# Wil-Lee/NN_BVH

Measured on AMD Instinct MI355X. Metric: Mray/s (closest-hit + any-hit), higher is better.
Workload: dtype f32; 1 GPU; crown, 1000x1400: one wavefront pass of 8 spp per step (8 spp per GPU-film) — primary, bounce-1 and bounce-2 closest-hit, shadow any-hit towards the light quads (batches pre-generated, hence independent: ONE launch; the dependent form is dependent_step), rays in --ray-order tile (a caller-side order the reference's integrator does not form: ray_order_probe), RecordShadowRayResult + RGBFilm::AddSam; sample_sets=4, geometry=procedural stand-in for crown (3548192 tris; data/crown.npz absent), tree=sah, triangles=3548192, nodes=7032259, rays_primary=11200000, rays_bounce=7410327, rays_bounce2=4392209, parallelism=tile-sharded x1, BVH replicated, film all-gather after the pass

## Files before the change

### nn_bvh_amd/aggregate.py

```python
import ctypes

import numpy as np

from . import _lib
from ._lib import HIT_DTYPE, NODE_DTYPE, PRIM_DTYPE, RAY_DTYPE, NNBVHError, check, ptr

SPLIT_METHODS = {"sah": 0, "hlbvh": 1, "middle": 2, "equal": 3}


def make_prims(tri_indices=None, patch_indices=None):
    nt = 0 if tri_indices is None else len(tri_indices)
    npch = 0 if patch_indices is None else len(patch_indices)
    prims = np.zeros(nt + npch, PRIM_DTYPE)
    prims["id"] = np.arange(nt + npch, dtype=np.int32)
    if nt:
        prims["kind"][:nt] = 0
        prims["v"][:nt, :3] = np.asarray(tri_indices, np.int32).reshape(nt, 3)
    if npch:
        prims["kind"][nt:] = 1
        prims["v"][nt:] = np.asarray(patch_indices, np.int32).reshape(npch, 4)
    return prims


def make_rays(o, d, tmax=np.inf, time=0.0):
# ... 313 lines not shown
            self.normals = np.ascontiguousarray(normals, np.float32).reshape(-1, 3)
            assert len(self.normals) == len(self.verts)
            self._h = L.nnbvh_scene_create_with_normals(ptr(self.nodes), len(self.nodes), ptr(self.ordered_prims),
                                                        len(self.ordered_prims), ptr(self.verts), ptr(self.normals),
                                                        len(self.verts), self.device)
        else:
            self._h = L.nnbvh_scene_create(ptr(self.nodes), len(self.nodes), ptr(self.ordered_prims),
                                           len(self.ordered_prims), ptr(self.verts), len(self.verts),
                                           self.device)
        if not self._h:
            raise NNBVHError("nnbvh_scene_create: " + _lib.last_error())
        self._read_info()

    def close(self):
        if getattr(self, "_h", None):
            _lib.lib().nnbvh_scene_destroy(self._h)
            self._h = None

    def __del__(self):
        try:
            self.close()
        except Exception:
            pass

    def set_option(self, key, value):
        check(_lib.lib().nnbvh_scene_set_option(self._h, key.encode(), int(value)),
              f"set_option({key})")

    def sched_stats(self, reset=True):
        out = np.zeros(16, np.uint64)
        check(_lib.lib().nnbvh_scene_sched_stats(self._h, ptr(out), int(reset)), "sched_stats")
        return dict(zip(("int_trips", "int_lanes", "prim_trips", "prim_lanes", "refill_trips",
                         "refill_lanes", "i_nint", "i_nprim", "i_nidle", "spare0", "int_cycles",
                         "prim_cycles", "refill_cycles", "spare1", "int_steps", "int_step_lanes"),
                        (int(x) for x in out)))

    def Bounds(self):
        out = np.zeros(6, np.float32)
        check(_lib.lib().nnbvh_scene_bounds(self._h, ptr(out)), "nnbvh_scene_bounds")
        return out[:3].copy(), out[3:].copy()

    def Intersect(self, rays, out=None):
        rays = np.ascontiguousarray(rays, RAY_DTYPE)
        hits = np.zeros(len(rays), HIT_DTYPE) if out is None else out
        assert hits.dtype == HIT_DTYPE and len(hits) == len(rays) and hits.flags.c_contiguous
        check(_lib.lib().nnbvh_intersect_closest(self._h, ptr(rays), len(rays), ptr(hits)),
              "nnbvh_intersect_closest")
        return hits

    def IntersectP(self, rays, counts=False):
        rays = np.ascontiguousarray(rays, RAY_DTYPE)
        occ = np.zeros(len(rays), np.uint8)
        if counts:
            vis = np.zeros(len(rays), np.int32)
            tst = np.zeros(len(rays), np.int32)
            check(_lib.lib().nnbvh_intersect_any(self._h, ptr(rays), len(rays), ptr(occ),
                                                 ptr(vis), ptr(tst)), "nnbvh_intersect_any")
            return occ, vis, tst
        check(_lib.lib().nnbvh_intersect_any(self._h, ptr(rays), len(rays), ptr(occ), None, None),
              "nnbvh_intersect_any")
        return occ

    def intersect_device(self, d_rays, d_hits, n, stream=0):
        check(_lib.lib().nnbvh_intersect_closest_device(self._h, d_rays, n, d_hits, stream),
              "nnbvh_intersect_closest_device")

    def trace_batches_device(self, batches, stream=0):
# ... 141 lines not shown
```

### nn_bvh_amd/build.py

```python
import concurrent.futures
import hashlib
import os
import shutil
import subprocess

HERE = os.path.dirname(os.path.abspath(__file__))
CSRC = os.path.join(HERE, "csrc")
LIB = os.path.join(HERE, "libnnbvh_hip.so")
SOURCES = ["bvh_trace.hip", "wavefront.hip", "wavefront2.hip", "wavefront_items.hip", "bvh_build_gpu.hip", "bvh_bake.hip", "interaction.hip", "film.hip", "kd_trace.hip", "kd_build_gpu.hip", "kd_bake.hip", "bvh_capi.cpp", "capi_two_level.cpp", "capi_trace.cpp", "capi_kd.cpp", "capi_wavefront.cpp", "capi_shading.cpp", "bvh_build.cpp", "kd_build.cpp"]
HEADERS = ["bvh_trace.h", "trace_instance.h", "trace_math.h", "stream_access.h", "spawn_math.h", "anim_math.h", "alpha_texture_math.h", "wavefront2.h", "walk_math.h", "wavefront.h", "bvh_build_gpu.h", "interaction.h", "interaction_math.h", "wavefront_items.h", "kd_trace.h", "kd_build_gpu.h", "kd_device_util.h", "nnbvh_internal.h", "capi_internal.h", os.path.join("..", "..", "include", "nnbvh.h")]
CFLAGS = ["-O3", "--offload-arch=gfx950", "-ffp-contract=off", "-fPIC", "-std=c++17",
          "-Wall", "-Wno-unused-function", "-Wno-pass-failed"]
FLAGS = CFLAGS + ["-shared"]


def _hipcc():
    hipcc = shutil.which("hipcc") or "/opt/rocm/bin/hipcc"
    if not os.path.exists(hipcc):
        raise RuntimeError("hipcc not found: cannot build libnnbvh_hip.so")
    return hipcc


def _sources():
    return [s for s in SOURCES if os.path.exists(os.path.join(CSRC, s))]


def _deps_mtime():
    deps = [os.path.join(CSRC, f) for f in HEADERS] + [os.path.abspath(__file__)]
    return max(os.path.getmtime(d) for d in deps if os.path.exists(d))


def _stale():
    if not os.path.exists(LIB):
        return True
    t = os.path.getmtime(LIB)
    return _deps_mtime() > t or any(os.path.getmtime(os.path.join(CSRC, s)) > t for s in _sources())


def _build(out, extra=(), force=False, verbose=False, jobs=None):
    hipcc = _hipcc()
    tag = hashlib.sha1(" ".join(extra).encode()).hexdigest()[:10] if extra else "product"
    objdir = os.path.join(HERE, "_obj", tag)
    os.makedirs(objdir, exist_ok=True)
# ... 43 lines not shown
```

### nn_bvh_amd/csrc/bvh_capi.cpp

```cpp
#include <algorithm>
#include <cmath>
#include <cstring>
#include <limits>
#include <vector>

#include "alpha_texture_math.h"
#include "bvh_build_gpu.h"
#include "capi_internal.h"

namespace nnbvh {

static thread_local std::string g_error;
void set_error(const std::string &msg) { g_error = msg; }

}

using namespace nnbvh;

static bool validate_tree(const nnbvh_linear_node *nodes, int root, int n_tree, const nnbvh_prim *prims,
                          int n_prims, bool allow_instances, std::vector<uint8_t> &covered,
                          std::vector<uint8_t> &leaf_last, int *depth_out) {
    if (n_tree < 1) {
        set_error("scene_create: tree has no nodes");
        return false;
    }
    const int n_nodes = root + n_tree;
    struct Frame {
        int node, end, depth;
    };
    std::vector<Frame> st;
    st.push_back({root, n_nodes, 0});
    int visited = 0, max_depth = 0;
    while (!st.empty()) {
        Frame f = st.back();
        st.pop_back();
        ++visited;
        if (f.node < 0 || f.node >= f.end) {
            set_error("scene_create: node index outside its subtree range");
            return false;
        }
        max_depth = std::max(max_depth, f.depth);
// ... 126 lines not shown
        AlphaTexDesc &d = table[(size_t)k];
        d.texelLo = (uint32_t)total;
        d.texelHi = (uint32_t)(total >> 32);
        d.width = t.width;
        d.height = t.height;
        d.wrap = t.wrap;
        d.pointFilter = t.point_filter ? 1 : 0;
        d.su = t.su, d.sv = t.sv, d.du = t.du, d.dv = t.dv;
        d.scale = t.scale;
        d.invert = t.invert ? 1 : 0;
        total += (uint64_t)t.width * (uint64_t)t.height;
    }
    DeviceGuard guard(s->device);
    bool ok = guard.ok && hip_ok(hipMalloc((void **)&s->d_alpha_tex, table.size() * sizeof(AlphaTexDesc)), "hipMalloc(alpha textures)") &&
              hip_ok(hipMalloc((void **)&s->d_alpha_texels, (size_t)total * 4), "hipMalloc(alpha texels)") &&
              hip_ok(hipMemcpy(s->d_alpha_tex, table.data(), table.size() * sizeof(AlphaTexDesc), hipMemcpyHostToDevice),
                     "hipMemcpy(alpha textures)");
    uint64_t at = 0;
    for (int k = 0; ok && k < n_textures; ++k) {
        const uint64_t n = (uint64_t)textures[k].width * (uint64_t)textures[k].height;
        ok = hip_ok(hipMemcpy(s->d_alpha_texels + at, textures[k].texels, (size_t)n * 4, hipMemcpyHostToDevice),
                    "hipMemcpy(alpha texels)");
        at += n;
    }
    if (!ok) {
        const std::string why = nnbvh_last_error();
        nnbvh_scene_destroy(s);
        set_error(why);
        return false;
    }
    s->n_alpha_tex = n_textures;
    s->n_alpha_texels = (int64_t)total;
    s->device_bytes += table.size() * sizeof(AlphaTexDesc) + (size_t)total * 4;
    return true;
}

extern "C" {

const char *nnbvh_last_error(void) { return g_error.c_str(); }

int nnbvh_device_count(void) {
    int n = 0;
    if (hipGetDeviceCount(&n) != hipSuccess) return 0;
    return n;
}

static nnbvh_scene *scene_from_baked(const BakedScene &b, int depth, int device) {
    hipDeviceProp_t prop;
    if (!hip_ok(hipGetDeviceProperties(&prop, device), "hipGetDeviceProperties")) {
        (void)hipFree(b.d_wide);
        return nullptr;
    }
    auto *s = new nnbvh_scene;
    s->device = device;
    s->n_cus = prop.multiProcessorCount;
    s->n_interior = b.n_interior;
    s->n_slots = b.n_slots;
    s->depth = depth;
    std::memcpy(s->bounds, b.bounds, sizeof b.bounds);
    s->root_ref = b.root_ref;
    s->instanced = 0;
    s->has_host_prims = (b.has_host_prims || b.has_alpha) ? 1 : 0;
    s->has_patches = (b.has_patches || b.has_alpha) ? 1 : 0;
    s->has_alpha = b.has_alpha;
    s->max_grid_threads = s->n_cus * 8 * kBlockThreads;
    s->d_wide = (float4 *)b.d_wide;
    s->d_prims = (float4 *)b.d_prims;
    s->device_bytes = (size_t)std::max(b.n_interior, 1) * sizeof(WideNode) +
                      std::max<size_t>((size_t)b.n_slots, 1) * 16;
    if (hipMalloc((void **)&s->d_stats, 16 * sizeof(unsigned long long)) == hipSuccess)
        (void)hipMemset(s->d_stats, 0, 16 * sizeof(unsigned long long));
    return s;
}

static nnbvh_scene *create_scene_device_bake(const nnbvh_linear_node *nodes, int n_nodes, const nnbvh_prim *prims,
                                             int n_prims, const float *verts, int n_verts, int depth, int device,
                                             const float *normals, const float *prim_alpha, const float *uvs) {
    int n_dev = nnbvh_device_count();
    if (n_dev <= 0 || device < 0 || device >= n_dev) {
        set_error("scene_create: no usable HIP device (this library has no CPU fallback)");
        return nullptr;
    }
    DeviceGuard guard(device);
    if (!guard.ok) return nullptr;
    void *d_nodes = nullptr, *d_prims = nullptr, *d_verts = nullptr, *d_normals = nullptr, *d_alpha = nullptr,
         *d_uvs = nullptr;
    const size_t nb = (size_t)n_nodes * sizeof(nnbvh_linear_node), pbytes = (size_t)n_prims * sizeof(nnbvh_prim),
                 vb = (size_t)n_verts * 12;
    BakedScene b;
    std::string err;
    bool ok = hip_ok(hipMalloc(&d_nodes, nb), "hipMalloc(tree)") && hip_ok(hipMalloc(&d_prims, pbytes), "hipMalloc(primitives)") &&
              hip_ok(hipMalloc(&d_verts, vb), "hipMalloc(vertices)") &&
              hip_ok(hipMemcpy(d_nodes, nodes, nb, hipMemcpyHostToDevice), "hipMemcpy(tree)") &&
              hip_ok(hipMemcpy(d_prims, prims, pbytes, hipMemcpyHostToDevice), "hipMemcpy(primitives)") &&
              hip_ok(hipMemcpy(d_verts, verts, vb, hipMemcpyHostToDevice), "hipMemcpy(vertices)");
    if (ok && normals)
        ok = hip_ok(hipMalloc(&d_normals, vb), "hipMalloc(normals)") &&
             hip_ok(hipMemcpy(d_normals, normals, vb, hipMemcpyHostToDevice), "hipMemcpy(normals)");
    if (ok && prim_alpha)
        ok = hip_ok(hipMalloc(&d_alpha, (size_t)n_prims * 4), "hipMalloc(primitive alpha)") &&
             hip_ok(hipMemcpy(d_alpha, prim_alpha, (size_t)n_prims * 4, hipMemcpyHostToDevice), "hipMemcpy(primitive alpha)");
    if (ok && uvs)
        ok = hip_ok(hipMalloc(&d_uvs, (size_t)n_verts * 8), "hipMalloc(uvs)") &&
             hip_ok(hipMemcpy(d_uvs, uvs, (size_t)n_verts * 8, hipMemcpyHostToDevice), "hipMemcpy(uvs)");
// ... 435 lines not shown
}

void nnbvh_scene_destroy(nnbvh_scene *s) {
    if (!s) return;
    DeviceGuard guard(s->device);
    (void)hipDeviceSynchronize();
    for (auto &kv : s->workspaces) {
        Workspace &w = kv.second;
        void *ptrs[] = {w.queue, w.spill, w.d_in, w.d_out, w.d_aux0, w.d_aux1, w.d_hits};
        for (void *p : ptrs)
            if (p) (void)hipFree(p);
        for (void *p : w.scratch)
            if (p) (void)hipFree(p);
    }
    for (HostSlot &sl : s->host_slots) {
        for (void *p : {sl.d_in, sl.d_out[0], sl.d_out[1], sl.d_out[2]})
            if (p) (void)hipFree(p);
        for (void *p : {sl.h_in, sl.h_out[0], sl.h_out[1], sl.h_out[2]})
            if (p) (void)hipHostFree(p);
        for (hipEvent_t e : {sl.ev_in, sl.ev_traced, sl.ev_out})
            if (e) (void)hipEventDestroy(e);
    }
    for (hipStream_t st : {s->host_up, s->host_trace, s->host_down})
        if (st) (void)hipStreamDestroy(st);
    for (int k = 0; k < nnbvh_scene::kSideStreams; ++k) {
        if (s->side[k]) (void)hipStreamDestroy(s->side[k]);
        if (s->ev_join[k]) (void)hipEventDestroy(s->ev_join[k]);
    }
    if (s->ev_fork) (void)hipEventDestroy(s->ev_fork);
    (void)hipFree(s->d_wide);
    if (s->d_anim) (void)hipFree(s->d_anim);
    if (s->d_alpha_tex) (void)hipFree(s->d_alpha_tex);
    if (s->d_alpha_texels) (void)hipFree(s->d_alpha_texels);
    if (s->d_stats) (void)hipFree(s->d_stats);
    delete s;
}

int nnbvh_scene_bounds(const nnbvh_scene *s, float out[6]) {
    if (!s || !out) {
        set_error("scene_bounds: null argument");
        return NNBVH_ERR_ARG;
    }
    std::memcpy(out, s->bounds, sizeof s->bounds);
    return NNBVH_OK;
}

int nnbvh_scene_info(const nnbvh_scene *s, int64_t out[6]) {
    if (!s || !out) {
        set_error("scene_info: null argument");
        return NNBVH_ERR_ARG;
    }
    out[0] = s->n_interior;
    out[1] = s->n_slots;
    out[2] = s->depth;
    out[3] = (int64_t)s->device_bytes;
    out[4] = grid_blocks(const_cast<nnbvh_scene *>(s), 0);
    out[5] = s->window;
    return NNBVH_OK;
}

int nnbvh_scene_read(const nnbvh_scene *s, int what, void *out, size_t bytes) {
    if (!s || !out) {
        set_error("scene_read: null argument");
        return NNBVH_ERR_ARG;
    }
    if (what < 0 || what > 4) {
// ... 64 lines not shown
    std::string k(key);
    if (k == "stack_window") {
        if (value != 4 && value != 8 && value != 16) {
            set_error("set_option: stack_window must be 4, 8 or 16");
            return NNBVH_ERR_ARG;
        }
        s->window = value;
    } else if (k == "blocks_per_cu") {
        if (value < 0 || value > 8) {
            set_error("set_option: blocks_per_cu must be 0..8");
            return NNBVH_ERR_ARG;
        }
        s->blocks_per_cu = value;
    } else if (k == "int_repeat") {
        if (value < 1 || value > 16) {
            set_error("set_option: int_repeat must be 1..16");
            return NNBVH_ERR_ARG;
        }
        s->int_repeat = value;
    } else if (k == "host_chunk") {
        if (value < 1024) {
            set_error("set_option: host_chunk must be at least 1024 rays");
            return NNBVH_ERR_ARG;
        }
        s->host_chunk = value;
    } else if (k == "prim_repeat") {
        if (value < 1 || value > 16) {
            set_error("set_option: prim_repeat must be 1..16");
            return NNBVH_ERR_ARG;
        }
        s->prim_repeat = value;
    } else if (k == "fused_batches") {
        s->fused_batches = value ? 1 : 0;
    } else if (k == "xcd_queues") {
        s->xcd_queues = value ? 1 : 0;
    } else if (k == "prim_weight") {
        if (value < 1 || value > 64) {
            set_error("set_option: prim_weight must be 1..64");
            return NNBVH_ERR_ARG;
        }
        s->prim_weight = value;
    } else if (k == "refill_weight") {
        if (value < 1 || value > 64) {
            set_error("set_option: refill_weight must be 1..64");
            return NNBVH_ERR_ARG;
        }
        s->refill_weight = value;
    } else {
        set_error("set_option: unknown key");
        return NNBVH_ERR_ARG;
    }
    return NNBVH_OK;
}

}

Workspace *nnbvh::workspace_for(nnbvh_scene *s, hipStream_t stream) {
    auto it = s->workspaces.find(stream);
    if (it != s->workspaces.end()) return &it->second;
    Workspace w;
    const size_t spill_bytes = (size_t)std::max(s->depth - 2, 1) * (size_t)s->max_grid_threads * sizeof(uint2);
    if (!hip_ok(hipMalloc((void **)&w.queue, kMaxFusedBatches * kMaxQueues * kQueueStrideWords * sizeof(unsigned)),
                "hipMalloc(queue)"))
        return nullptr;
    if (!hip_ok(hipMalloc((void **)&w.spill, spill_bytes), "hipMalloc(spill)")) {
        (void)hipFree(w.queue);
// ... 5 lines not shown
```

### nn_bvh_amd/csrc/bvh_trace.h

```cpp
#pragma once
#include <hip/hip_runtime.h>
#include <stdint.h>

#include "../../include/nnbvh.h"
#include "nnbvh_internal.h"
#include "trace_instance.h"
#include "walk_math.h"

namespace nnbvh {

constexpr int kBlockThreads = 256;
constexpr int kMaxQueues = 8;
constexpr int kQueueStrideWords = 32;
constexpr int kMaxFusedBatches = 4;
constexpr int kFusedIndexBits = 28;

struct TraceParams {
    const float4 *wide;
    const float4 *prims;
    float rootMin[3], rootMax[3];
    int rootRef;
    const nnbvh_ray *rays;
    nnbvh_hit *hits;
    uint8_t *occluded;
// ... 4 lines not shown
    unsigned *queue;
    int nQueues;
    int primWeight;
    int refillWeight;
    int hasHostPrims;
    int intRepeat;
    int primRepeat;
    int fits32;
    unsigned long long *stats;
    uint2 *spill;
    const float *anim;
    int nBatches;
    unsigned anyMask;
    const nnbvh_ray *bRays[kMaxFusedBatches];
    void *bOut[kMaxFusedBatches];
    long bN[kMaxFusedBatches];
    const int32_t *bNDev[kMaxFusedBatches];
    nnbvh_ray_soa soa;
    nnbvh_ray_soa bSoa[kMaxFusedBatches];
    int hcCap;
    int32_t *hcCount;
    int32_t *hcBefore;
    int32_t *hcPrim;
    int32_t *hcInst;
    int bHcCap[kMaxFusedBatches];
    int32_t *bHcCount[kMaxFusedBatches];
    int32_t *bHcBefore[kMaxFusedBatches];
    int32_t *bHcPrim[kMaxFusedBatches];
    int32_t *bHcInst[kMaxFusedBatches];
    ShadingMeshDevice wMesh;
    WalkParams walk;
    const float4 *alphaTex;
    const float *alphaTexels;
};

hipError_t launch_zero_queue(unsigned *queue, int words, hipStream_t stream);
hipError_t launch_zero_words(int32_t *words, long n, int maxBlocks, hipStream_t stream);

hipError_t launch_trace(const TraceInstance &is, const TraceParams &p, int blocks, hipStream_t stream, int *occupancy);

}
```

### nn_bvh_amd/csrc/bvh_trace.hip

```cpp
#include <hip/hip_runtime.h>
#include <stdint.h>
#include <array>
#include <cstring>
#include <utility>

#include "bvh_trace.h"
#include "alpha_texture_math.h"
#include "anim_math.h"
#include "spawn_math.h"
#include "stream_access.h"
#include "trace_math.h"
#include "walk_math.h"

namespace nnbvh {

constexpr int kDone = (int)0x80000000;
constexpr int kReturn = (int)0x80000001;
constexpr int kEnter = (int)0x80000002;

#ifndef NNBVH_MINW_CLOSEST
#define NNBVH_MINW_CLOSEST 6
#endif
#ifndef NNBVH_MINW_ANY
#define NNBVH_MINW_ANY 6
// ... 16 lines not shown
#ifndef NNBVH_MINW_WALK
#define NNBVH_MINW_WALK 4
#endif
constexpr int min_waves(int modew, int inst, int patch, int alpha) {
    if (inst) return 1;
    if (modew >= 4) return patch ? NNBVH_MINW_WALK : NNBVH_MINW_WALK_LEAN;
    if (alpha == 2) return NNBVH_MINW_ALPHA_PATCH;
    if (alpha == 3) return NNBVH_MINW_ALPHA_TEX;
    if (alpha) return NNBVH_MINW_ALPHA;
    return ((modew == 0 || modew == 3) ? NNBVH_MINW_CLOSEST : NNBVH_MINW_ANY) + (patch ? 0 : NNBVH_LEAN_EXTRA_WAVES);
}
#ifndef NNBVH_ANIM_ENTER_WEIGHT
#define NNBVH_ANIM_ENTER_WEIGHT 8
#endif
template <typename T>
__device__ __forceinline__ T pick_batch(const T (&a)[kMaxFusedBatches], int b) {
    static_assert(kMaxFusedBatches == 4, "written out for four batches");
    return b == 0 ? a[0] : (b == 1 ? a[1] : (b == 2 ? a[2] : a[3]));
}

#define BVH_BEGIN_RAY(R0, R1)                                                                                         \
    do {                                                                                                              \
        r.o = {(R0).x, (R0).y, (R0).z};                                                                               \
        tMax = (R0).w;                                                                                                \
        const V3 d = {(R1).x, (R1).y, (R1).z};                                                                        \
        if (PATCH) {                                                                                                  \
            cold[kColdD][lane] = d.x;                                                                                 \
            cold[kColdD + 1][lane] = d.y;                                                                             \
            cold[kColdD + 2][lane] = d.z;                                                                             \
        }                                                                                                             \
                                                                                          \
        r.inv = {1.0f / d.x, 1.0f / d.y, 1.0f / d.z};                                                                 \
        ray_shear(r, d);                                                                                              \
        if (MODE == 0 || MODE == 3) {                                                                                 \
            cold[kColdHit][lane] = __int_as_float(-1);                                                                \
            cold[kColdHit + 1][lane] = 0.0f;                                                                          \
            cold[kColdHit + 2][lane] = 0.0f;                                                                          \
            cold[kColdHit + 3][lane] = 0.0f;                                                                          \
        }                                                                                                             \
        if (INST) {                                                                                                   \
            cold[kHitInst][lane] = 0.0f;                                                                              \
            cold[kCurInst][lane] = 0.0f;                                                                              \
            cold[kColdTime][lane] = (R1).w;                                 \
            floor = -1;                                                                                               \
        }                                                                                                             \
        if (!kLean && (HOSTC || p.hasHostPrims)) cold[kColdHost][lane] = 0.0f;           \
        if constexpr (WALK != 0) {                                                                                    \
            cold[kWalkD][lane] = (R1).x;                                                                              \
            cold[kWalkD + 1][lane] = (R1).y;                                                                          \
            cold[kWalkD + 2][lane] = (R1).z;                                                                          \
            cold[kWalkTime][lane] = (R1).w;                                                                           \
            cold[kWalkTMax][lane] = (R0).w;                                                                           \
        }                                                                                                             \
        visited = 1;                                                                                    \
        tests = 0;                                                                                                    \
        found = false;                                                                                                \
        sp = base = 0;                                                                                                \
        float tEntry;                                                                                                 \
        const bool rootHit = slab_partial(p.rootMin[0], p.rootMin[1], p.rootMin[2], p.rootMax[0], p.rootMax[1],       \
                                          p.rootMax[2], r, tEntry) &&                                                 \
                             (tEntry < tMax);                                                                         \
        cur = rootHit ? p.rootRef : kDone;                                                                            \
    } while (0)

template <int MODEW, int W, int INST, int PATCH, int ALPHA = 0, int SOA = 0, int HOSTC = 0>
__global__ __launch_bounds__(kBlockThreads, min_waves(MODEW, INST, PATCH, ALPHA))
void trace_kernel(TraceParams p) {
    constexpr int WALK = MODEW >= 4 ? MODEW - 3 : 0;
    constexpr int MODE = WALK ? 0 : MODEW;
    static_assert(!WALK || (MODEW <= 5 && W == 8 && INST != 2 && !ALPHA && !SOA && !HOSTC),
                  "walk instances: the plain record-reading closest-hit form at window 8");
    static_assert(PATCH || !INST, "two-level scenes need the ray direction");
    static_assert(PATCH || !ALPHA, "the alpha test hashes the ray direction");
    static_assert(ALPHA != 3 || (INST == 0 && W == 8 && MODE != 3), "textured alpha: flat scenes, window 8, modes 0 / 1 / 2");
    static_assert(!HOSTC || (PATCH && (MODE == 0 || MODE == 2 || (MODE == 3 && !ALPHA && W == 8)) && !SOA),
                  "candidate mode: general instances of modes 0 / 2 / 3");
    __shared__ float s_stack[kBlockThreads / 64][W][2][64];
    constexpr bool kLean = !PATCH && !INST;
    constexpr int kColdRi = 0, kColdD = 1, kColdHit = kLean ? 0 : (PATCH ? 4 : 1),
                  kColdHost = kColdHit + ((MODE == 0 || MODE == 3) ? 4 : 0);
    constexpr int kColdBase = kColdHost + (kLean ? 0 : 1);
    constexpr int kSaveO = kColdBase, kSaveInv = kColdBase + 3, kSaveShear = kColdBase + 6,
                  kSaveKz = kColdBase + 9, kSaveTmax = kColdBase + 10, kSaveD = kColdBase + 11,
                  kResume = kColdBase + 14, kCurInst = kColdBase + 15, kHitInst = kColdBase + 16,
                  kInnerHit = kColdBase + 17, kColdTime = kColdBase + 18, kPendSlot = kColdBase + 19;
    constexpr int kColdWalk = kColdBase + (INST ? 20 : 0);
    [[maybe_unused]] constexpr int kWalkD = kColdWalk, kWalkTime = kColdWalk + 3, kWalkTMax = kColdWalk + 4,
                                   kWalkCalls = kColdWalk + 5;
    constexpr int kColdFields = kColdWalk + (WALK ? 6 : 0);
    __shared__ float s_cold[kBlockThreads / 64][kColdFields > 0 ? kColdFields : 1][64];

    const int lane = threadIdx.x & 63;
    const int wave = threadIdx.x >> 6;
    const int gtid = blockIdx.x * kBlockThreads + threadIdx.x;
    float(*stk)[2][64] = s_stack[wave];
    float(*cold)[64] = s_cold[wave];
    int riReg = -1;
    if (!kLean) cold[kColdRi][lane] = __int_as_float(-1);
    const long spillStride = (long)gridDim.x * kBlockThreads;

    int q = 0;
    if (p.nQueues > 1) {
        unsigned xcc;
        asm volatile("s_getreg_b32 %0, hwreg(HW_REG_XCC_ID)" : "=s"(xcc));
        q = (int)(xcc & 0xf) % p.nQueues;
    }
    int queuesTried = 0;
    int curBatch = 0;
    long nRays = p.n;
    if (p.nDev) {
        const long nd = (long)*p.nDev;
        nRays = nd < 0 ? 0 : (nd < nRays ? nd : nRays);
    }

#ifdef NNBVH_STATS
    unsigned long long st[16] = {0, 0, 0, 0, 0, 0, 0, 0, 0, 0, 0, 0, 0, 0, 0, 0};
    unsigned long long stPrev = __builtin_amdgcn_s_memtime();
    int stKind = 2;
#endif
    RayState r;
    RayMasks masks = {0ull, 0ull, 0ull, 0ull, 0ull, 0ull};
    float tMax = 0.0f;
    int visited = 0, tests = 0;
    int cur = kDone, sp = 0, base = 0;
    int floor = -1;
    bool found = false;
    bool exhausted = false;

    auto pop_entry = [&](int &ref, float &key) {
// ... 188 lines not shown
                        const float u = (a <= 0) ? 1.f : hash_float_6f(rn.o, rd);
                        if (!(u > a)) break;
                        if (k == kAlphaPatchDepth) {
                            hit = false;
                            cold[kColdHost][lane] = HOSTC ? __int_as_float(-2) : 1.0f;
                            break;
                        }
                        if (k == 0) t0 = th;
                        else if (k == 1) t1 = th;
                        else t2 = th;
                        ++k;
                        rn.o = patch_retrace_origin({s0.x, s0.y, s0.z}, {s1.x, s1.y, s1.z}, {s2.x, s2.y, s2.z},
                                                    {s3.x, s3.y, s3.z}, x0, x1, (flags & kPrimFlipN) != 0, rd,
                                                    (flags & kPrimSmooth) != 0, (flags & kPrimUV) != 0,
                                                    p.prims + slot + 4);
                        tm = tm - th;
                        tests += 1;
                    }
                    if (hit && k > 0) {
                        if (k == 3) th = th + t2;
                        if (k >= 2) th = th + t1;
                        th = th + t0;
                    }
                } else {
                    hit = patch_test(r, rd, tMax, {s0.x, s0.y, s0.z}, {s1.x, s1.y, s1.z},
                                     {s2.x, s2.y, s2.z}, {s3.x, s3.y, s3.z}, x0, x1, th);
                }
            }
            bool closestLane = MODE == 0;
            if (MODE == 3 && hit)
                closestLane = !((p.anyMask >> ((kLean ? riReg : __float_as_int(cold[kColdRi][lane])) >> kFusedIndexBits)) & 1u);
            if (hit) {
                if (closestLane) {
                    cold[kColdHit][lane] = s0.w;
                    cold[kColdHit + 1][lane] = x0;
                    cold[kColdHit + 2][lane] = x1;
                    cold[kColdHit + 3][lane] = x2;
                    tMax = th;
                    if (INST) {
                        cold[kHitInst][lane] = cold[kCurInst][lane];
                        cold[kInnerHit][lane] = 1.0f;
                    }
                    if constexpr (HOSTC && MODE == 0) {
                        const int c = __float_as_int(cold[kColdHost][lane]);
                        if (c > 0) p.hcBefore[__float_as_int(cold[kColdRi][lane])] = c;
                    }
                    if constexpr (HOSTC && MODE == 3) {
                        const int c = __float_as_int(cold[kColdHost][lane]);
                        if (c > 0) {
                            const int tag = __float_as_int(cold[kColdRi][lane]);
                            pick_batch(p.bHcBefore, tag >> kFusedIndexBits)[tag & ((1 << kFusedIndexBits) - 1)] = c;
                        }
                    }
                } else {
                    found = true;
                }
            }
            if (MODE != 0 && found) cur = kDone;
            else if (flags & kPrimLast) cur = pop_next();
            else cur = ~next;
        }
    };

    auto interior_math = [&](const float4 q0, const float4 q1, const float4 q2, const float4 q3) {
        const int ref0 = __float_as_int(q3.x), ref1 = __float_as_int(q3.y);
        const int axis = __float_as_int(q3.z);
        const bool swap = ((r.kz >> axis) & 1) != 0;
        const float k0 = kLean ? slab_entry_key(q0.x, q0.y, q0.z, q0.w, q1.x, q1.y, r, masks)
                               : slab_entry_key(q0.x, q0.y, q0.z, q0.w, q1.x, q1.y, r);
        const float k1 = kLean ? slab_entry_key(q1.z, q1.w, q2.x, q2.y, q2.z, q2.w, r, masks)
                               : slab_entry_key(q1.z, q1.w, q2.x, q2.y, q2.z, q2.w, r);
        const int nearRef = swap ? ref1 : ref0, farRef = swap ? ref0 : ref1;
        const float nearT = swap ? k1 : k0, farT = swap ? k0 : k1;
        visited += 1;
        const bool doPush = (MODE == 1) || (farT < __builtin_inff());
        if (doPush && sp - base == W - 1) {
            uint2 e;
            e.x = __float_as_uint(stk[base & (W - 1)][0][lane]);
            e.y = __float_as_uint(stk[base & (W - 1)][1][lane]);
            p.spill[(long)base * spillStride + gtid] = e;
            ++base;
        }
        stk[sp & (W - 1)][0][lane] = __int_as_float(farRef);
        stk[sp & (W - 1)][1][lane] = farT;
        sp += doPush ? 1 : 0;
        if (MODE == 0 || MODE == 3) visited += doPush ? 0 : 1;
        cur = nearT < tMax ? nearRef : pop_next();
    };
    auto interior_step = [&]() {
#ifdef NNBVH_STATS
        st[14] += 1;
        st[15] += __popcll(__ballot(cur >= 0));
#endif
        if (cur >= 0) {
            const float4 *rec = kLean ? reinterpret_cast<const float4 *>(reinterpret_cast<const char *>(p.wide) + ((unsigned)cur << 6))
                                      : p.wide + 4 * (long)cur;
            const float4 q3 = rec[3];
            const float4 q0 = rec[0], q1 = rec[1], q2 = rec[2];
            interior_math(q0, q1, q2, q3);
        }
    };

    for (;;) {
#ifdef NNBVH_STATS
        {
            const unsigned long long now = __builtin_amdgcn_s_memtime();
            st[10 + stKind] += now - stPrev;
            stPrev = now;
        }
#endif
        const bool isInt = cur >= 0;
        const bool isIdle = cur == kDone;
        const int nInt = __popcll(__ballot(isInt));
        const unsigned long long idleMask = __ballot(isIdle);
        const int nIdle = __popcll(idleMask);
        const int nEnter = (INST == 2 && NNBVH_ANIM_ENTER_WEIGHT > 0) ? __popcll(__ballot(cur == kEnter)) : 0;
        const int nPrim = 64 - nInt - nIdle - nEnter;

        const int sI = nInt * 16, sP = nPrim * p.primWeight;
        const int sR = exhausted ? 0 : nIdle * p.refillWeight;
#ifdef NNBVH_STATS
        unsigned long long &stTrips = (nIdle == 64 || (sR > sI && sR > sP)) ? st[4]
                                      : ((sP > sI || nInt == 0) ? st[2] : st[0]);
        (&stTrips)[0] += 1;
        (&stTrips)[1] += (nIdle == 64 || (sR > sI && sR > sP)) ? nIdle
                         : ((sP > sI || nInt == 0) ? nPrim : nInt);
        stKind = (&stTrips == &st[4]) ? 2 : ((&stTrips == &st[2]) ? 1 : 0);
// ... 48 lines not shown
                if (ri >= 0) {
                    const int b = ri >> kFusedIndexBits;
                    const long idx = ri & ((1 << kFusedIndexBits) - 1);
                    void *outp = pick_batch(p.bOut, b);
                    const int c = __float_as_int(cold[kColdHost][lane]);
                    if (pick_batch(p.bHcCap, b) > 0) pick_batch(p.bHcCount, b)[idx] = c;
                    if ((p.anyMask >> b) & 1u) {
                        store_stream(reinterpret_cast<uint8_t *>(outp) + idx, (uint8_t)(found ? 1 : (c != 0 ? 2 : 0)));
                    } else {
                        float4 h0, h1;
                        h0.x = cold[kColdHit][lane];
                        h0.y = tMax;
                        h0.z = cold[kColdHit + 1][lane];
                        h0.w = cold[kColdHit + 2][lane];
                        h1.x = cold[kColdHit + 3][lane];
                        h1.y = __int_as_float(visited);
                        h1.z = __int_as_float(tests);
                        h1.w = INST ? cold[kHitInst][lane] : 0.0f;
                        if (c < 0) h1.w = __int_as_float(-1);
                        float4 *out = reinterpret_cast<float4 *>(outp) + 2 * idx;
                        store_stream(out, h0);
                        store_stream(out + 1, h1);
                    }
                }
            } else if (MODE == 3 && ri >= 0) {
                const int b = ri >> kFusedIndexBits;
                const long idx = ri & ((1 << kFusedIndexBits) - 1);
                void *outp = b == 0 ? p.bOut[0] : (b == 1 ? p.bOut[1] : (b == 2 ? p.bOut[2] : p.bOut[3]));
                const bool needHost = !kLean && p.hasHostPrims && cold[kColdHost][lane] != 0.0f;
                if ((p.anyMask >> b) & 1u) {
                    store_stream(reinterpret_cast<uint8_t *>(outp) + idx, (uint8_t)(found ? 1 : (needHost ? 2 : 0)));
                } else {
                    float4 h0, h1;
                    h0.x = cold[kColdHit][lane];
                    h0.y = tMax;
                    h0.z = cold[kColdHit + 1][lane];
                    h0.w = cold[kColdHit + 2][lane];
                    h1.x = cold[kColdHit + 3][lane];
                    h1.y = __int_as_float(visited);
                    h1.z = __int_as_float(tests);
                    h1.w = INST ? cold[kHitInst][lane] : 0.0f;
                    if (needHost) h1.w = __int_as_float(-1);
                    float4 *out = reinterpret_cast<float4 *>(outp) + 2 * idx;
                    store_stream(out, h0);
                    store_stream(out + 1, h1);
                }
            } else if (ri >= 0) {
                if (MODE == 0) {
                    float4 h0, h1;
                    h0.x = cold[kColdHit][lane];
                    h0.y = tMax;
                    h0.z = cold[kColdHit + 1][lane];
                    h0.w = cold[kColdHit + 2][lane];
                    h1.x = cold[kColdHit + 3][lane];
                    h1.y = __int_as_float(visited);
                    h1.z = __int_as_float(tests);
                    h1.w = INST ? cold[kHitInst][lane] : 0.0f;
                    if constexpr (HOSTC) {
                        const int c = __float_as_int(cold[kColdHost][lane]);
                        if (c < 0) h1.w = __int_as_float(-1);
                        p.hcCount[ri] = c;
                    } else if (!kLean && p.hasHostPrims && cold[kColdHost][lane] != 0.0f) {
                        h1.w = __int_as_float(-1);
                    }
                    float4 *out = reinterpret_cast<float4 *>(p.hits) + 2 * (long)ri;
                    store_stream(out, h0);
                    store_stream(out + 1, h1);
                } else {
                    bool needHost;
                    if constexpr (HOSTC) {
                        const int c = __float_as_int(cold[kColdHost][lane]);
// ... 209 lines not shown
```

### nn_bvh_amd/csrc/capi_internal.h

```cpp
#pragma once
#include <hip/hip_runtime.h>

#include <cstddef>
#include <cstdint>
#include <map>
#include <mutex>
#include <string>
#include <type_traits>

#include "bvh_trace.h"
#include "interaction.h"
#include "kd_trace.h"

namespace nnbvh {

inline bool hip_ok(hipError_t e, const char *what) {
    if (e == hipSuccess) return true;
    set_error(std::string(what) + ": " + hipGetErrorString(e));
    return false;
}

struct DeviceGuard {
    int prev = -1;
    bool ok = false;
// ... 41 lines not shown
    float *d_anim = nullptr;
    int n_anim = 0;
    size_t device_bytes = 0;
    int window = 8;
    int blocks_per_cu = 0;
    int xcd_queues = 1;
    int prim_weight = 32;
    int refill_weight = 8;
    unsigned long long *d_stats = nullptr;
    int instanced = 0;
    int has_host_prims = 0;
    int has_patches = 1;
    int has_alpha = 0;
    int fused_batches = 1;
    int int_repeat = 3;
    int prim_repeat = 2;
    int max_grid_threads = 0;
    int walk_blocks_per_cu[6] = {0, 0, 0, 0, 0, 0};
    double build_ms[1] = {0};
    std::mutex mu;
    std::map<hipStream_t, nnbvh::Workspace> workspaces;
    static constexpr int kHostSlots = 3, kHostChunks = 6;
    nnbvh::HostSlot host_slots[kHostSlots];
    hipStream_t host_up = nullptr, host_trace = nullptr, host_down = nullptr;
    int64_t host_chunk = 1 << 20;
    static constexpr int kSideStreams = 4;
    hipStream_t side[kSideStreams] = {nullptr, nullptr, nullptr, nullptr};
    hipEvent_t ev_fork = nullptr;
    hipEvent_t ev_join[kSideStreams] = {nullptr, nullptr, nullptr, nullptr};
    void *d_alpha_tex = nullptr;
    float *d_alpha_texels = nullptr;
    int n_alpha_tex = 0;
    int64_t n_alpha_texels = 0;
};

struct nnbvh_shading_mesh {
    int device = 0;
    int n_cus = 0;
    nnbvh::ShadingMeshDevice d;
};

namespace nnbvh {

Workspace *workspace_for(nnbvh_scene *s, hipStream_t stream);

void fill_anim_entry(const nnbvh_animated_transform &a, float *t);

inline KdWorkspace *workspace_for(nnbvh_kd_scene *s, hipStream_t stream) { return kd_workspace_for(s, stream); }

template <class S, class W = std::remove_pointer_t<decltype(workspace_for((S *)nullptr, hipStream_t()))>>
struct SceneCall {
    DeviceGuard guard;
    std::unique_lock<std::mutex> lock;
    W *w = nullptr;
    bool good;
    explicit SceneCall(S *s) : guard(s->device), good(guard.ok) {
        if (good) lock = std::unique_lock<std::mutex>(s->mu);
    }
    SceneCall(S *s, hipStream_t stream) : SceneCall(s) {
        if (good) good = (w = workspace_for(s, stream)) != nullptr;
    }
    bool ok() const { return good; }
};

inline bool grow(void **ptr, size_t *have, size_t need, const char *what) {
    if (*have >= need) return true;
// ... 79 lines not shown
```

### nn_bvh_amd/csrc/capi_trace.cpp

```cpp
#include <algorithm>
#include <cstring>
#include <thread>

#include "capi_internal.h"

using namespace nnbvh;

int nnbvh::grid_blocks(nnbvh_scene *s, int mode, int candidates) {
    int per_cu = s->blocks_per_cu;
    if (per_cu <= 0) {
        TraceInstance is{};
        if (!pick_trace_instance(scene_traits(s), mode, candidates > 0, false, &is) ||
            launch_trace(is, TraceParams{}, 0, nullptr, &per_cu) != hipSuccess || per_cu <= 0)
            per_cu = std::max(1, std::min(8, 160 / (s->window * 2)));
    }
    per_cu = std::min(per_cu, 8);
    return s->n_cus * per_cu;
}

bool nnbvh::zero_candidates(int n_cus, const nnbvh_host_candidates *hc, int64_t n, bool closest, hipStream_t stream) {
    return hip_ok(launch_zero_words(hc->count, (long)n, n_cus * 8, stream), "candidate count reset launch") &&
           (!closest || !hc->before ||
            hip_ok(launch_zero_words(hc->before, (long)n, n_cus * 8, stream), "candidate before reset launch"));
}
// ... 98 lines not shown
int nnbvh::launch_fused_batches(nnbvh_scene *s, Workspace *w, hipStream_t stream, const nnbvh_batch *batches,
                                int n_batches, const int32_t *const *d_n, const nnbvh_ray_soa *const *soas,
                                const nnbvh_host_candidates *cands) {
    TraceParams p = scene_params(s, w);
    int64_t total = 0;
    bool candidates = false, soa = false;
    for (int i = 0; i < n_batches; ++i) {
        if (batches[i].n == 0) continue;
        const int b = p.nBatches++;
        p.bRays[b] = (const nnbvh_ray *)batches[i].d_rays;
        soa = soa || !batches[i].d_rays;
        p.bOut[b] = batches[i].d_out;
        p.bN[b] = (long)batches[i].n;
        p.bNDev[b] = d_n ? d_n[i] : nullptr;
        if (soas && soas[i]) p.bSoa[b] = *soas[i];
        if (batches[i].kind == NNBVH_BATCH_ANY) p.anyMask |= 1u << b;
        total += batches[i].n;
        if (cands && cands[i].capacity > 0) {
            const bool closest = batches[i].kind == NNBVH_BATCH_CLOSEST;
            if (!zero_candidates(s->n_cus, &cands[i], batches[i].n, closest, stream)) return NNBVH_ERR_DEVICE;
            if (s->has_host_prims) {
                candidates = true;
                p.hcCap = 1;
                p.bHcCap[b] = cands[i].capacity;
                p.bHcCount[b] = cands[i].count;
                p.bHcBefore[b] = closest ? cands[i].before : nullptr;
                p.bHcPrim[b] = cands[i].prim;
                p.bHcInst[b] = cands[i].instance;
            }
        }
    }
    if (p.nBatches == 0) return NNBVH_OK;
    p.n = (long)total;
    return run_trace(s, stream, 3, candidates, soa, p, kMaxFusedBatches * kMaxQueues * kQueueStrideWords,
                     "fused trace kernel launch");
}

bool nnbvh::batches_fusable(const nnbvh_scene *s, const nnbvh_batch *batches, int n_batches) {
    bool fusable = s->fused_batches && n_batches <= kMaxFusedBatches && s->window == 8 && !s->has_alpha;
    for (int i = 0; fusable && i < n_batches; ++i)
        fusable = batches[i].n < (1LL << kFusedIndexBits) &&
                  !(batches[i].kind == NNBVH_BATCH_ANY && (batches[i].d_nodes_visited || batches[i].d_prim_tests));
    return fusable;
}

const char *nnbvh::candidates_fault(const nnbvh_host_candidates *c, bool closest) {
    if (!c) return "candidates is NULL";
    if (c->capacity < 1 || c->capacity > 16) return "capacity must be 1..16";
    if (!c->count || !c->prim || !c->instance) return "count, prim and instance are required";
    if (closest && !c->before) return "before is required for closest hit";
    return nullptr;
}

bool nnbvh::candidates_ok(const char *fn, const nnbvh_host_candidates *c, bool closest) {
    const char *why = candidates_fault(c, closest);
    if (why) set_error(std::string(fn) + ": " + why);
    return !why;
}

static bool batch_args_ok(const char *fn, const nnbvh_scene *s, int64_t n, const void *rays, const void *out,
                          const char *candidates_wrong = nullptr) {
    const char *why = nullptr;
    if (!s || n < 0 || (n > 0 && (!rays || !out))) why = "bad argument";
    else if (candidates_wrong) why = candidates_wrong;
    else if (n >= 0x7fffffffLL) why = "at most 2^31-1 rays per call";
    if (why) set_error(std::string(fn) + ": " + why);
// ... 355 lines not shown
```

### nn_bvh_amd/csrc/nnbvh_internal.h

```cpp
#pragma once
#include <cstdint>
#include <string>

#include "../../include/nnbvh.h"

namespace nnbvh {

void set_error(const std::string &msg);
const char *candidates_fault(const nnbvh_host_candidates *c, bool closest);

struct WideNode {
    float q[12];
    int32_t ref0, ref1;
    int32_t axis;
    int32_t pad;
};
static_assert(sizeof(WideNode) == 64, "WideNode must be 64 bytes");

constexpr uint32_t kPrimLast = 1u;
constexpr uint32_t kPrimPatch = 2u;
constexpr uint32_t kPrimDegenerate = 4u;
constexpr uint32_t kPrimInstance = 8u;
constexpr uint32_t kPrimHost = 16u;

// ... 1 lines not shown
constexpr uint32_t kPrimFlipN = 64u;
constexpr uint32_t kPrimAnimated = 128u;
constexpr uint32_t kPrimSmooth = 256u;
constexpr uint32_t kPrimUV = 512u;
constexpr uint32_t kPrimAlphaTex = 1024u;
constexpr int kAnimStride = 76;
constexpr bool is_triangle_kind(int kind) {
    return kind == NNBVH_PRIM_TRIANGLE || kind == NNBVH_PRIM_ALPHA_TRIANGLE || kind == NNBVH_PRIM_ALPHA_TRIANGLE_FLIPPED ||
           kind == NNBVH_PRIM_ALPHA_TRIANGLE_SMOOTH || kind == NNBVH_PRIM_ALPHA_TRIANGLE_SMOOTH_FLIPPED;
}
constexpr bool is_smooth_alpha_kind(int kind) {
    return kind == NNBVH_PRIM_ALPHA_TRIANGLE_SMOOTH || kind == NNBVH_PRIM_ALPHA_TRIANGLE_SMOOTH_FLIPPED;
}
constexpr bool is_alpha_patch_kind(int kind) { return kind >= NNBVH_PRIM_ALPHA_PATCH && kind <= NNBVH_PRIM_ALPHA_PATCH_UV_SMOOTH_FLIPPED; }
constexpr bool is_smooth_alpha_patch_kind(int kind) { return is_alpha_patch_kind(kind) && ((kind - NNBVH_PRIM_ALPHA_PATCH) & 2); }
constexpr bool is_flipped_alpha_patch_kind(int kind) { return is_alpha_patch_kind(kind) && ((kind - NNBVH_PRIM_ALPHA_PATCH) & 1); }
constexpr bool is_uv_alpha_patch_kind(int kind) { return is_alpha_patch_kind(kind) && ((kind - NNBVH_PRIM_ALPHA_PATCH) & 4); }
constexpr int alpha_patch_slots(int kind) { return 4 + (is_smooth_alpha_patch_kind(kind) ? 4 : 0) + (is_uv_alpha_patch_kind(kind) ? 2 : 0); }
constexpr bool is_flat_alpha_kind(int kind) {
    return kind == NNBVH_PRIM_ALPHA_TRIANGLE || kind == NNBVH_PRIM_ALPHA_TRIANGLE_FLIPPED;
}

constexpr bool is_alphatex_kind(int kind) { return kind >= NNBVH_PRIM_ALPHATEX_TRIANGLE && kind <= NNBVH_PRIM_ALPHATEX_TRIANGLE_SMOOTH_FLIPPED; }
constexpr bool is_smooth_alphatex_kind(int kind) { return is_alphatex_kind(kind) && ((kind - NNBVH_PRIM_ALPHATEX_TRIANGLE) & 2); }
constexpr bool is_flipped_alphatex_kind(int kind) { return is_alphatex_kind(kind) && ((kind - NNBVH_PRIM_ALPHATEX_TRIANGLE) & 1); }
constexpr int alphatex_slots(int kind) { return 5 + (is_smooth_alphatex_kind(kind) ? 3 : 0); }
constexpr int kMaxAlphaTexSize = 1 << 24;
constexpr const char *kAlphaTexElsewhere =
    "unknown primitive kind (image-textured alpha, kinds 16 .. 19, is for flat BVH scenes: "
    "nnbvh_scene_create_with_alpha_textures / nnbvh_scene_create_gpu_build_with_alpha_textures)";

constexpr int kMaxStack = 64;

#if defined(__HIPCC__)
#define NNBVH_HD __host__ __device__
#else
#define NNBVH_HD
#endif
NNBVH_HD inline float kd_difference_of_products(float a, float b, float c, float d) {
    const float cd = c * d;
    const float diff = __builtin_fmaf(a, b, -cd);
    const float err = __builtin_fmaf(-c, d, cd);
    return diff + err;
}
NNBVH_HD inline bool kd_triangle_is_degenerate(const float *p0, const float *p1, const float *p2) {
    const float v[3] = {p2[0] - p0[0], p2[1] - p0[1], p2[2] - p0[2]};
    const float w[3] = {p1[0] - p0[0], p1[1] - p0[1], p1[2] - p0[2]};
    const float cx = kd_difference_of_products(v[1], w[2], v[2], w[1]);
    const float cy = kd_difference_of_products(v[2], w[0], v[0], w[2]);
    const float cz = kd_difference_of_products(v[0], w[1], v[1], w[0]);
    return cx * cx + cy * cy + cz * cz == 0.0f;
}

NNBVH_HD inline void transform_bounds(const float m[12], const float in[6], float out[6]) {
    float mn[3], mx[3];
    for (int k = 0; k < 3; ++k) {
        mn[k] = 3.402823466e+38f;
        mx[k] = -3.402823466e+38f;
    }
    for (int c = 0; c < 8; ++c) {
        const float p[3] = {in[(c & 1) ? 3 : 0], in[(c & 2) ? 4 : 1], in[(c & 4) ? 5 : 2]};
        for (int k = 0; k < 3; ++k) {
            const float v = m[4 * k] * p[0] + m[4 * k + 1] * p[1] + m[4 * k + 2] * p[2] + m[4 * k + 3];
            mn[k] = v < mn[k] ? v : mn[k];
            mx[k] = mx[k] < v ? v : mx[k];
        }
// ... 9 lines not shown
```

Measured before the change: 4786 Mray/s.

## Cache top BVH levels in LDS and keep closest-hit record in registers

```diff
diff --git a/nn_bvh_amd/aggregate.py b/nn_bvh_amd/aggregate.py
--- a/nn_bvh_amd/aggregate.py
+++ b/nn_bvh_amd/aggregate.py
@@ -369,7 +369,7 @@
         check(_lib.lib().nnbvh_scene_sched_stats(self._h, ptr(out), int(reset)), "sched_stats")
         return dict(zip(("int_trips", "int_lanes", "prim_trips", "prim_lanes", "refill_trips",
                          "refill_lanes", "i_nint", "i_nprim", "i_nidle", "spare0", "int_cycles",
-                         "prim_cycles", "refill_cycles", "spare1", "int_steps", "int_step_lanes"),
+                         "prim_cycles", "refill_cycles", "int_top_lanes", "int_steps", "int_step_lanes"),
                         (int(x) for x in out)))
 
     def Bounds(self):
diff --git a/nn_bvh_amd/build.py b/nn_bvh_amd/build.py
--- a/nn_bvh_amd/build.py
+++ b/nn_bvh_amd/build.py
@@ -8,7 +8,7 @@
 CSRC = os.path.join(HERE, "csrc")
 LIB = os.path.join(HERE, "libnnbvh_hip.so")
 SOURCES = ["bvh_trace.hip", "wavefront.hip", "wavefront2.hip", "wavefront_items.hip", "bvh_build_gpu.hip", "bvh_bake.hip", "interaction.hip", "film.hip", "kd_trace.hip", "kd_build_gpu.hip", "kd_bake.hip", "bvh_capi.cpp", "capi_two_level.cpp", "capi_trace.cpp", "capi_kd.cpp", "capi_wavefront.cpp", "capi_shading.cpp", "bvh_build.cpp", "kd_build.cpp"]
-HEADERS = ["bvh_trace.h", "trace_instance.h", "trace_math.h", "stream_access.h", "spawn_math.h", "anim_math.h", "alpha_texture_math.h", "wavefront2.h", "walk_math.h", "wavefront.h", "bvh_build_gpu.h", "interaction.h", "interaction_math.h", "wavefront_items.h", "kd_trace.h", "kd_build_gpu.h", "kd_device_util.h", "nnbvh_internal.h", "capi_internal.h", os.path.join("..", "..", "include", "nnbvh.h")]
+HEADERS = ["bvh_trace.h", "trace_instance.h", "top_table.h", "trace_math.h", "stream_access.h", "spawn_math.h", "anim_math.h", "alpha_texture_math.h", "wavefront2.h", "walk_math.h", "wavefront.h", "bvh_build_gpu.h", "interaction.h", "interaction_math.h", "wavefront_items.h", "kd_trace.h", "kd_build_gpu.h", "kd_device_util.h", "nnbvh_internal.h", "capi_internal.h", os.path.join("..", "..", "include", "nnbvh.h")]
 CFLAGS = ["-O3", "--offload-arch=gfx950", "-ffp-contract=off", "-fPIC", "-std=c++17",
           "-Wall", "-Wno-unused-function", "-Wno-pass-failed"]
 FLAGS = CFLAGS + ["-shared"]
diff --git a/nn_bvh_amd/csrc/bvh_capi.cpp b/nn_bvh_amd/csrc/bvh_capi.cpp
--- a/nn_bvh_amd/csrc/bvh_capi.cpp
+++ b/nn_bvh_amd/csrc/bvh_capi.cpp
@@ -7,6 +7,7 @@
 #include "alpha_texture_math.h"
 #include "bvh_build_gpu.h"
 #include "capi_internal.h"
+#include "top_table.h"
 
 namespace nnbvh {
 
@@ -199,6 +200,25 @@
     s->n_alpha_tex = n_textures;
     s->n_alpha_texels = (int64_t)total;
     s->device_bytes += table.size() * sizeof(AlphaTexDesc) + (size_t)total * 4;
+    return true;
+}
+
+static bool attach_top_table(nnbvh_scene *s) {
+    if (!scene_runs_lean(s)) return true;
+    std::vector<WideNode> table;
+    std::vector<int32_t> order;
+    const auto fetch = [&](int32_t record, WideNode *out) {
+        return hip_ok(hipMemcpy(out, s->d_wide + 4 * (size_t)record, sizeof(WideNode), hipMemcpyDeviceToHost),
+                      "hipMemcpy(top record)");
+    };
+    if (!build_top_table(fetch, s->root_ref, s->n_interior, kTopRecords, &table, &order)) return false;
+    if (table.empty()) return true;
+    const size_t bytes = table.size() * sizeof(WideNode);
+    if (!hip_ok(hipMalloc((void **)&s->d_top, bytes), "hipMalloc(top table)") ||
+        !hip_ok(hipMemcpy(s->d_top, table.data(), bytes, hipMemcpyHostToDevice), "hipMemcpy(top table)"))
+        return false;
+    s->n_top = (int)table.size();
+    s->device_bytes += bytes;
     return true;
 }
 
@@ -237,6 +257,12 @@
                       std::max<size_t>((size_t)b.n_slots, 1) * 16;
     if (hipMalloc((void **)&s->d_stats, 16 * sizeof(unsigned long long)) == hipSuccess)
         (void)hipMemset(s->d_stats, 0, 16 * sizeof(unsigned long long));
+    if (!attach_top_table(s)) {
+        const std::string why = nnbvh_last_error();
+        nnbvh_scene_destroy(s);
+        set_error(why);
+        return nullptr;
+    }
     return s;
 }
 
@@ -738,6 +764,7 @@
     if (s->d_anim) (void)hipFree(s->d_anim);
     if (s->d_alpha_tex) (void)hipFree(s->d_alpha_tex);
     if (s->d_alpha_texels) (void)hipFree(s->d_alpha_texels);
+    if (s->d_top) (void)hipFree(s->d_top);
     if (s->d_stats) (void)hipFree(s->d_stats);
     delete s;
 }
@@ -868,6 +895,8 @@
         s->prim_repeat = value;
     } else if (k == "fused_batches") {
         s->fused_batches = value ? 1 : 0;
+    } else if (k == "top_table") {
+        s->use_top = value ? 1 : 0;
     } else if (k == "xcd_queues") {
         s->xcd_queues = value ? 1 : 0;
     } else if (k == "prim_weight") {
diff --git a/nn_bvh_amd/csrc/bvh_trace.h b/nn_bvh_amd/csrc/bvh_trace.h
--- a/nn_bvh_amd/csrc/bvh_trace.h
+++ b/nn_bvh_amd/csrc/bvh_trace.h
@@ -60,6 +60,8 @@
     WalkParams walk;
     const float4 *alphaTex;
     const float *alphaTexels;
+    const float4 *top;
+    int nTop;
 };
 
 hipError_t launch_zero_queue(unsigned *queue, int words, hipStream_t stream);
diff --git a/nn_bvh_amd/csrc/bvh_trace.hip b/nn_bvh_amd/csrc/bvh_trace.hip
--- a/nn_bvh_amd/csrc/bvh_trace.hip
+++ b/nn_bvh_amd/csrc/bvh_trace.hip
@@ -72,7 +72,10 @@
                                                                                           \
         r.inv = {1.0f / d.x, 1.0f / d.y, 1.0f / d.z};                                                                 \
         ray_shear(r, d);                                                                                              \
-        if (MODE == 0 || MODE == 3) {                                                                                 \
+        if constexpr (kTop) {                                                                                         \
+            hit0 = __int_as_float(-1);                                                                                \
+            hit1 = hit2 = hit3 = 0.0f;                                                                                \
+        } else if (MODE == 0 || MODE == 3) {                                                                          \
             cold[kColdHit][lane] = __int_as_float(-1);                                                                \
             cold[kColdHit + 1][lane] = 0.0f;                                                                          \
             cold[kColdHit + 2][lane] = 0.0f;                                                                          \
@@ -128,13 +131,25 @@
     [[maybe_unused]] constexpr int kWalkD = kColdWalk, kWalkTime = kColdWalk + 3, kWalkTMax = kColdWalk + 4,
                                    kWalkCalls = kColdWalk + 5;
     constexpr int kColdFields = kColdWalk + (WALK ? 6 : 0);
-    __shared__ float s_cold[kBlockThreads / 64][kColdFields > 0 ? kColdFields : 1][64];
+    constexpr bool kTop = kLean && MODEW == 3;
 
     const int lane = threadIdx.x & 63;
     const int wave = threadIdx.x >> 6;
     const int gtid = blockIdx.x * kBlockThreads + threadIdx.x;
     float(*stk)[2][64] = s_stack[wave];
-    float(*cold)[64] = s_cold[wave];
+    float(*cold)[64] = nullptr;
+    [[maybe_unused]] const float4 *top = nullptr;
+    if constexpr (kTop) {
+        __shared__ float4 s_top[kTopRecords * 4];
+        static_assert(kTopRecords * 4 <= kBlockThreads, "one float4 per thread copies the table");
+        if ((int)threadIdx.x < p.nTop * 4) s_top[threadIdx.x] = p.top[threadIdx.x];
+        __syncthreads();
+        top = s_top;
+    } else {
+        __shared__ float s_cold[kBlockThreads / 64][kColdFields > 0 ? kColdFields : 1][64];
+        cold = s_cold[wave];
+    }
+    [[maybe_unused]] float hit0 = 0.0f, hit1 = 0.0f, hit2 = 0.0f, hit3 = 0.0f;
     int riReg = -1;
     if (!kLean) cold[kColdRi][lane] = __int_as_float(-1);
     const long spillStride = (long)gridDim.x * kBlockThreads;
@@ -389,10 +404,17 @@
                 closestLane = !((p.anyMask >> ((kLean ? riReg : __float_as_int(cold[kColdRi][lane])) >> kFusedIndexBits)) & 1u);
             if (hit) {
                 if (closestLane) {
-                    cold[kColdHit][lane] = s0.w;
-                    cold[kColdHit + 1][lane] = x0;
-                    cold[kColdHit + 2][lane] = x1;
-                    cold[kColdHit + 3][lane] = x2;
+                    if constexpr (kTop) {
+                        hit0 = s0.w;
+                        hit1 = x0;
+                        hit2 = x1;
+                        hit3 = x2;
+                    } else {
+                        cold[kColdHit][lane] = s0.w;
+                        cold[kColdHit + 1][lane] = x0;
+                        cold[kColdHit + 2][lane] = x1;
+                        cold[kColdHit + 3][lane] = x2;
+                    }
                     tMax = th;
                     if (INST) {
                         cold[kHitInst][lane] = cold[kCurInst][lane];
@@ -448,8 +470,27 @@
 #ifdef NNBVH_STATS
         st[14] += 1;
         st[15] += __popcll(__ballot(cur >= 0));
-#endif
-        if (cur >= 0) {
+        if (kTop) st[13] += __popcll(__ballot(cur >= 0 && (cur & kTopTag) != 0));
+#endif
+        if constexpr (kTop) {
+            if (cur >= 0) {
+                typedef float v4f __attribute__((ext_vector_type(4)));
+                const unsigned at = (unsigned)cur << 6;
+                v4f q0, q1, q2, q3;
+                if (cur & kTopTag) {
+                    const v4f *rec = reinterpret_cast<const v4f *>(reinterpret_cast<const char *>(top) + at);
+                    q3 = rec[3];
+                    q0 = rec[0], q1 = rec[1], q2 = rec[2];
+                    asm volatile("" : "+v"(q0), "+v"(q1), "+v"(q2), "+v"(q3));
+                } else {
+                    const v4f *rec = reinterpret_cast<const v4f *>(reinterpret_cast<const char *>(p.wide) + at);
+                    q3 = rec[3];
+                    q0 = rec[0], q1 = rec[1], q2 = rec[2];
+                }
+                interior_math({q0.x, q0.y, q0.z, q0.w}, {q1.x, q1.y, q1.z, q1.w}, {q2.x, q2.y, q2.z, q2.w},
+                              {q3.x, q3.y, q3.z, q3.w});
+            }
+        } else if (cur >= 0) {
             const float4 *rec = kLean ? reinterpret_cast<const float4 *>(reinterpret_cast<const char *>(p.wide) + ((unsigned)cur << 6))
                                       : p.wide + 4 * (long)cur;
             const float4 q3 = rec[3];
@@ -564,11 +605,11 @@
                     store_stream(reinterpret_cast<uint8_t *>(outp) + idx, (uint8_t)(found ? 1 : (needHost ? 2 : 0)));
                 } else {
                     float4 h0, h1;
-                    h0.x = cold[kColdHit][lane];
+                    h0.x = kTop ? hit0 : cold[kColdHit][lane];
                     h0.y = tMax;
-                    h0.z = cold[kColdHit + 1][lane];
-                    h0.w = cold[kColdHit + 2][lane];
-                    h1.x = cold[kColdHit + 3][lane];
+                    h0.z = kTop ? hit1 : cold[kColdHit + 1][lane];
+                    h0.w = kTop ? hit2 : cold[kColdHit + 2][lane];
+                    h1.x = kTop ? hit3 : cold[kColdHit + 3][lane];
                     h1.y = __int_as_float(visited);
                     h1.z = __int_as_float(tests);
                     h1.w = INST ? cold[kHitInst][lane] : 0.0f;
diff --git a/nn_bvh_amd/csrc/capi_internal.h b/nn_bvh_amd/csrc/capi_internal.h
--- a/nn_bvh_amd/csrc/capi_internal.h
+++ b/nn_bvh_amd/csrc/capi_internal.h
@@ -97,6 +97,9 @@
     float *d_alpha_texels = nullptr;
     int n_alpha_tex = 0;
     int64_t n_alpha_texels = 0;
+    float4 *d_top = nullptr;
+    int n_top = 0;
+    int use_top = 1;
 };
 
 struct nnbvh_shading_mesh {
diff --git a/nn_bvh_amd/csrc/capi_trace.cpp b/nn_bvh_amd/csrc/capi_trace.cpp
--- a/nn_bvh_amd/csrc/capi_trace.cpp
+++ b/nn_bvh_amd/csrc/capi_trace.cpp
@@ -154,6 +154,11 @@
     }
     if (p.nBatches == 0) return NNBVH_OK;
     p.n = (long)total;
+    if (s->d_top && s->use_top && !candidates && scene_runs_lean(s)) {
+        p.top = s->d_top;
+        p.nTop = s->n_top;
+        p.rootRef = kTopTag;
+    }
     return run_trace(s, stream, 3, candidates, soa, p, kMaxFusedBatches * kMaxQueues * kQueueStrideWords,
                      "fused trace kernel launch");
 }
diff --git a/nn_bvh_amd/csrc/nnbvh_internal.h b/nn_bvh_amd/csrc/nnbvh_internal.h
--- a/nn_bvh_amd/csrc/nnbvh_internal.h
+++ b/nn_bvh_amd/csrc/nnbvh_internal.h
@@ -57,6 +57,9 @@
 
 constexpr int kMaxStack = 64;
 
+constexpr int kTopRecords = 63;
+constexpr int32_t kTopTag = 1 << 30;
+
 #if defined(__HIPCC__)
 #define NNBVH_HD __host__ __device__
 #else
diff --git a/nn_bvh_amd/csrc/top_table.h b/nn_bvh_amd/csrc/top_table.h
--- /dev/null
+++ b/nn_bvh_amd/csrc/top_table.h
@@ -0,0 +1,30 @@
+#pragma once
+#include <cstdint>
+#include <vector>
+
+#include "nnbvh_internal.h"
+
+namespace nnbvh {
+
+template <class Fetch>
+bool build_top_table(Fetch fetch, int32_t root_ref, int n_interior, int capacity, std::vector<WideNode> *table,
+                     std::vector<int32_t> *order) {
+    table->clear();
+    order->clear();
+    if (root_ref < 0 || root_ref >= n_interior || capacity < 1) return true;
+    order->push_back(root_ref);
+    for (size_t k = 0; k < order->size(); ++k) {
+        WideNode w;
+        if (!fetch((*order)[k], &w)) return false;
+        for (int32_t *ref : {&w.ref0, &w.ref1}) {
+            if (*ref < 0 || *ref >= n_interior || (int)order->size() >= capacity) continue;
+            const int32_t slot = (int32_t)order->size();
+            order->push_back(*ref);
+            *ref = kTopTag | slot;
+        }
+        table->push_back(w);
+    }
+    return true;
+}
+
+}
```

Result: faster. 4869 Mray/s, median of 6 (+1.8%).
